# AtlasAnalyticsLab/AtlasPatch

Measured on AMD Instinct MI355X. Metric: patches/sec embedded (256x256, ViT-B/16), higher is better.
Workload: dtype f16

## Files before the change

atlaspatch_amd/csrc/ap_common.h:

```cpp
#pragma once
#include <hip/hip_runtime.h>
#include <cstdarg>
#include <cstdint>
#include <cstdio>
#include "../../include/atlaspatch_hip.h"

namespace ap {

void set_error(const char* fmt, ...);

#define AP_HIP_CHECK(expr)                                                              \
    do {                                                                                \
        hipError_t _e = (expr);                                                         \
        if (_e != hipSuccess) {                                                         \
            ap::set_error("%s failed: %s (%s:%d)", #expr, hipGetErrorString(_e),        \
                          __FILE__, __LINE__);                                          \
            return AP_ERR_HIP;                                                          \
        }                                                                               \
    } while (0)

#define AP_REQUIRE(cond, ...)                                                           \
    do {                                                                                \
        if (!(cond)) {                                                                  \
            ap::set_error(__VA_ARGS__);                                                 \
// ... 90 lines not shown
    int split;
    const float* resid; int ldr;
    int win_mode, win_ws, win_H, win_W, win_nwy, win_nwx;
    const float* zero_row;
};
void set_gemm_trace(long long* buf, int tiles_per_wg);

int launch_gemm(int dtype, int epilogue, const GemmArgs& a, hipStream_t stream);
int launch_gemm_impl(int dtype, int epilogue, const GemmArgs& a, int impl, int variant, hipStream_t stream);
bool gemm256_supports(int dtype, int epilogue, const GemmArgs& a);
int launch_gemm256(int dtype, int epilogue, const GemmArgs& a, int variant, hipStream_t stream);
int launch_gemm256_alt(int dtype, int epilogue, const GemmArgs& a, int variant, hipStream_t stream);

int launch_layernorm(int dtype, const float* x, long stride, int rows, int dim,
                     const float* gamma, const float* beta, float eps, void* out,
                     hipStream_t stream);
int launch_add_layernorm(int delta_dtype, int out_dtype, float* x, long stride, const void* delta,
                         long dstride, const float* ls, int rows, int dim, const float* gamma, const float* beta,
                         float eps, void* out, hipStream_t stream);
int launch_add2_layernorm(int delta_dtype, int out_dtype, float* x, long stride, const void* delta0, long dstride0,
                          const float* ls0, const void* delta1, long dstride1, const float* ls1, int store,
                          int rows, int dim, const float* gamma, const float* beta, float eps, void* out,
                          hipStream_t stream);
int launch_layernorm_f32out(const float* x, long stride, int rows, int dim, const float* gamma,
                            const float* beta, float eps, float* out, hipStream_t stream);
int launch_attention(int dtype, const void* qkv, void* out, int n, int tokens, int heads,
                     int head_dim, float scale, hipStream_t stream);
int launch_attention_flash(int dtype, const void* qkv, void* out, int n, int tokens, int heads, int head_dim, float scale,
                           hipStream_t stream);
int launch_attention_cls(int dtype, const void* q, const void* kv, int ld, int koff, int voff, void* out, int n,
                         int tokens, int heads, int head_dim, float scale, hipStream_t stream);
int launch_attn_pool(int dtype, const void* kv, const float* q, void* out, int n, int tokens, int heads,
                     hipStream_t stream);
int launch_stream_init(int dtype, const float* tok, int rows, int dim, float eps, void* x, float* rowstats,
                       hipStream_t stream);
int launch_rowstats_finalize(const float* partial, int rows, int groups, int dim, float eps, float* rowstats,
                             hipStream_t stream);
int launch_rowstats_finalize_cls(const float* partial, int rows, int groups, int dim, float eps, float* rowstats, int dtype,
                                 float* cls32, const float* branch, void* x, int n, int tokens, hipStream_t stream);
int launch_stream_to_f32(int dtype, const void* x, long stride, int rows, int dim, float* dst, hipStream_t stream);
int launch_rope(int dtype, void* qkv, int n, int tokens, int prefix, int heads, int head_dim, const float* cos, const float* sin,
                int which, hipStream_t stream);
int launch_cls_mean_pool(const float* y, int n, int tokens, int prefix, int dim, float* out, hipStream_t stream);
int launch_fold_ln(int dtype, const float* w32, int rows, int cols, int ld, const float* gamma, const float* beta,
                   const float* bias_in, void* wout, float* colsum, float* bias_out, hipStream_t stream, int swiglu_h = 0);
int launch_fold_ls(int dtype, const float* w32, int rows, int cols, int ld, const float* ls, const float* bias_in,
                   void* wout, float* bias_out, hipStream_t stream);
int launch_cls_stream(int dtype, const float* prefix, int prefix_rows, int img_rows, int n, int tokens, int dim, void* x, float* partial,
                      hipStream_t stream);
int launch_cls_init(float* tok, const float* prefix, int prefix_rows, int n, int tokens, int dim, hipStream_t stream);
int launch_cls_exact_update(int dtype, float* cls32, const float* branch, int n, int tokens, int dim, void* x, float* partial,
                            hipStream_t stream);
int launch_swiglu(int dtype, const void* x, int rows, int h, void* out, hipStream_t stream);
int launch_prefix_build(const float* cls, const float* reg, int reg_rows, const float* pos, int dim, float* prefix, hipStream_t stream);
int launch_convert(int dtype, const float* src, void* dst, size_t count, hipStream_t stream);
int launch_split_f16_weights(const float* src, void* dst, size_t count, hipStream_t stream);
int launch_chw_to_patchrows(int x_dtype, int dtype, const void* x, int n, int S, int ps, void* dst,
                            int ld, hipStream_t stream);

bool sattention_supports(int heads, int tq, int tk, int d, long ldq, long ldk, long ldv, long ldo);
int launch_sattention(const float* q, long ldq, const float* k, long ldk, const float* v, long ldv, int batch, int heads, int tq,
                      int tk, int d, float scale, float* out, long ldo, hipStream_t stream, bool exact);

int launch_conv2d_nhwc(int dtype, const void* x, int n, int h, int w, int cin, const void* weight, const float* bias, int cout,
                       int ksize, int stride, int pad, const void* resid, int relu, void* out, hipStream_t stream);
int launch_preproc_nhwc8(const uint8_t* src, int n, int h, int w, int top, int left, int S, const float mean[3],
// ... 27 lines not shown
```

atlaspatch_amd/csrc/vit.cpp:

```cpp
#include <cmath>
#include <cstdlib>
#include <cstring>
#include <map>
#include <string>
#include <vector>
#include "engine_host.h"

namespace ap {

struct Param {
    size_t count = 0;
    int rows = 0, cols = 0, ld = 0;
    bool matrix = false;
    void* dev = nullptr;
    float* dev32 = nullptr;
    void* split = nullptr;
    bool set = false;
};

struct BlockParams {
    const float *ln1_w, *ln1_b, *qkv_b, *proj_b, *ln2_w, *ln2_b, *fc1_b, *fc2_b, *ls1, *ls2;
    const Param *qkv, *proj, *fc1, *fc2;
};
struct FusedBlock {
    void *qkv_w = nullptr, *fc1_w = nullptr, *proj_w = nullptr, *fc2_w = nullptr;
    float *qkv_cs = nullptr, *qkv_b = nullptr, *fc1_cs = nullptr, *fc1_b = nullptr, *proj_b = nullptr, *fc2_b = nullptr;
};
struct PoolParams {
    const float *ln_k_w, *ln_k_b, *kv_b, *q, *out_b, *ln_out_w, *ln_out_b;
    const Param *kv, *out;
};
}

struct ap_vit {
    ap_vit_config cfg;
    int grid = 0, patches = 0, tokens = 0, kpe = 0;
    int prefix = 1;
    int pos_rows = 0, pos_row0 = 1;
    int hd = 64, dattn = 0;
    int fc1_rows = 0;
    float attn_scale = 0.125f;
    float* prefix_dev = nullptr;
    std::map<std::string, ap::Param> params;
    bool finalized = false;
    std::vector<ap::BlockParams> blocks;
    ap::PoolParams pool{};
    const ap::Param* pe_w = nullptr;
    const float *pe_b = nullptr, *cls = nullptr, *pos = nullptr, *norm_w = nullptr, *norm_b = nullptr;
    const float *pre_w = nullptr, *pre_b = nullptr;
    const float *rope_cos = nullptr, *rope_sin = nullptr;
    const ap::Param* head_proj = nullptr;
    float* zero_bias = nullptr;
    bool full_last_block = false, two_half_overlap = false, f32_stream = false;
    bool exact_cls = true;
    bool split_f16 = false;
    std::vector<ap::FusedBlock> fused;
    std::vector<void*> fused_allocs;
    void* pos16 = nullptr;
    bool fold_dirty = false;
    std::vector<float*> pending_free;
    int device = 0;
    ap::LaunchProfiler prof;
    hipStream_t side = nullptr;
    hipEvent_t ev_fork = nullptr, ev_join = nullptr;

    ~ap_vit() {
        for (auto& kv : params) {
            if (kv.second.dev) (void)hipFree(kv.second.dev);
            if (kv.second.dev32) (void)hipFree(kv.second.dev32);
            if (kv.second.split) (void)hipFree(kv.second.split);
        }
        for (void* p : fused_allocs) (void)hipFree(p);
        if (prefix_dev) (void)hipFree(prefix_dev);
        if (zero_bias) (void)hipFree(zero_bias);
        if (ev_fork) (void)hipEventDestroy(ev_fork);
        if (ev_join) (void)hipEventDestroy(ev_join);
        if (side) (void)hipStreamDestroy(side);
    }
};

namespace {

using ap::Param;
using ap::ScopedTimer;

int alloc_param(ap_vit* m, const std::string& name, int rows, int cols, bool matrix) {
    Param p;
// ... 88 lines not shown
      if ((rc = ap::launch_gemm(dt, ap::EPI_PATCH_EMBED, g, stream)) != AP_OK) return rc; }
    return ap::launch_cls_init(w.tok, m->prefix_dev, m->prefix, n, m->tokens, D, stream);
}

int patch_embed_stream(ap_vit* m, int n, const Workspace& w, hipStream_t stream) {
    const ap_vit_config& c = m->cfg;
    const int dt = c.compute_dtype, D = c.dim;
    int rc;
    ap::GemmArgs g{};
    g.A = w.hid; g.lda = m->kpe; set_weight(m, g, m->pe_w);
    g.M = n * m->patches; g.N = D; g.K = m->kpe;
    g.bias = m->pe_b; g.pos16 = m->pos16; g.P = m->patches; g.R = m->prefix; g.pos_row0 = m->pos_row0;
    g.out = w.x16; g.ldo = D; g.partial = w.partial;
    { ScopedTimer t(m->prof, AP_PROF_GEMM_PATCH_EMBED, stream);
      if ((rc = ap::launch_gemm(dt, ap::EPI_PATCH_STREAM, g, stream)) != AP_OK) return rc; }
    ScopedTimer t(m->prof, AP_PROF_LAYERNORM, stream);
    if ((rc = ap::launch_cls_stream(dt, m->prefix_dev, m->prefix, 0, n, m->tokens, D, w.x16, w.partial, stream)) != AP_OK) return rc;
    return ap::launch_rowstats_finalize(w.partial, n * m->tokens, D / 64, D, c.ln_eps, w.rowstats, stream);
}

int block_attention(ap_vit* m, int n, const Workspace& w, hipStream_t stream) {
    const ap_vit_config& c = m->cfg;
    const int DA = m->dattn;
    ScopedTimer t(m->prof, AP_PROF_ATTENTION, stream);
    if (use_split(m) && n <= 65535) {
        const float* qp = (const float*)w.qkv;
        return ap::launch_sattention(qp, 3 * DA, qp + DA, 3 * DA, qp + 2 * DA, 3 * DA, n, c.heads, m->tokens, m->tokens, m->hd,
                                     m->attn_scale, (float*)w.att, DA, stream, false);
    }
    return ap::launch_attention(c.compute_dtype, w.qkv, w.att, n, m->tokens, c.heads, m->hd, m->attn_scale, stream);
}

int cls_tail_rows(ap_vit* m, int n, const Workspace& w, const ap::BlockParams& bp, long xn_stride, long tok_stride,
                  const void* pending, const float* pending_ls, long pending_stride, hipStream_t stream) {
    const ap_vit_config& c = m->cfg;
    const int dt = c.compute_dtype, D = c.dim, DA = m->dattn, H = c.mlp_dim, F1 = m->fc1_rows;
    const bool swiglu = c.mlp_type == AP_MLP_SWIGLU;
    int rc;
    char* q_cls = (char*)w.att;
    char* a_cls = (char*)w.att + (size_t)n * DA * ap::dtype_size(dt);
    {
        ap::GemmArgs g{};
        g.A = w.xn; g.lda = (int)xn_stride; set_weight(m, g, bp.qkv);
        g.M = n; g.N = DA; g.K = D; g.bias = bp.qkv_b; g.out = q_cls; g.ldo = DA;
        if ((rc = ap::launch_gemm_impl(dt, ap::EPI_BIAS_STORE, g, 128, 0, stream)) != AP_OK) return rc;
    }
    if ((rc = ap::launch_attention_cls(dt, q_cls, w.qkv, 3 * DA, DA, 2 * DA, a_cls, n, m->tokens, c.heads,
                                       m->hd, m->attn_scale, stream)) != AP_OK) return rc;
    {
        ap::GemmArgs g{};
        g.A = a_cls; g.lda = DA; set_weight(m, g, bp.proj);
        g.M = n; g.N = D; g.K = DA; g.bias = bp.proj_b; g.out = w.delta2; g.ldo = D;
        if ((rc = ap::launch_gemm_impl(dt, ap::EPI_BIAS_STORE, g, 128, 0, stream)) != AP_OK) return rc;
    }
    if ((rc = ap::launch_add2_layernorm(dt, dt, w.tok, tok_stride, pending, pending_stride, pending_ls, w.delta2, D,
                                        bp.ls1, 1, n, D, bp.ln2_w, bp.ln2_b, c.ln_eps, w.xn, stream)) != AP_OK)
        return rc;
    {
        ap::GemmArgs g{};
        g.A = w.xn; g.lda = D; set_weight(m, g, bp.fc1);
        g.M = n; g.N = F1; g.K = D; g.bias = bp.fc1_b; g.out = w.hid; g.ldo = F1;
        if ((rc = ap::launch_gemm_impl(dt, fc1_epilogue(c, false), g, 128, 0, stream)) != AP_OK) return rc;
        if (swiglu && (rc = ap::launch_swiglu(dt, w.hid, n, H, w.hid2, stream)) != AP_OK) return rc;
    }
    ap::GemmArgs g{};
    g.A = w.hid2; g.lda = H; set_weight(m, g, bp.fc2);
    g.M = n; g.N = D; g.K = H; g.bias = bp.fc2_b; g.out = w.delta; g.ldo = D;
    return ap::launch_gemm_impl(dt, ap::EPI_BIAS_STORE, g, 128, 0, stream);
}

int blocks_f32_stream(ap_vit* m, int n, const Workspace& w, StreamTail& st, hipStream_t stream) {
    const ap_vit_config& c = m->cfg;
    const int dt = c.compute_dtype, D = c.dim, M = n * m->tokens;
    const int DA = m->dattn, H = c.mlp_dim, F1 = m->fc1_rows;
    const bool swiglu = c.mlp_type == AP_MLP_SWIGLU;
    int rc;
    const void* pending = nullptr;
    long pending_stride = D;
    const bool cls_tail = c.pool == AP_POOL_CLS && !m->full_last_block;
    const float* pending_ls = nullptr;
    for (int i = 0; i < c.depth; ++i) {
// ... 60 lines not shown
    st.pending_stride = cls_tail ? pending_stride : (long)m->tokens * D;
    return AP_OK;
}

int blocks_fused(ap_vit* m, int n, const Workspace& w, StreamTail& st, hipStream_t stream) {
    const ap_vit_config& c = m->cfg;
    const int dt = c.compute_dtype, D = c.dim, M = n * m->tokens, G = D / 64;
    const int DA = m->dattn, H = c.mlp_dim, F1 = m->fc1_rows;
    const bool swiglu = c.mlp_type == AP_MLP_SWIGLU;
    int rc;
    const bool cls_tail = c.pool == AP_POOL_CLS && !m->full_last_block;
    const bool exact_cls = m->exact_cls && (c.pool == AP_POOL_CLS || c.pool == AP_POOL_CLS_MEAN) && M < (1 << 24);
    const long cls_stride = (long)m->tokens;
    if (exact_cls) {
        ScopedTimer t(m->prof, AP_PROF_CLS_TAIL, stream);
        if (c.pre_norm) {
            AP_HIP_CHECK(hipMemcpy2DAsync(w.cls32, (size_t)D * 4, w.tok, (size_t)cls_stride * D * 4, (size_t)D * 4, n,
                                          hipMemcpyDeviceToDevice, stream));
        } else if ((rc = ap::launch_cls_init(w.cls32, m->prefix_dev, 1, n, 1, D, stream)) != AP_OK) return rc;
    }
    auto exact_cls_update = [&]() -> int {
        ScopedTimer t(m->prof, AP_PROF_LAYERNORM, stream);
        return ap::launch_cls_exact_update(dt, w.cls32, w.cls_branch, n, m->tokens, D, w.x16, w.partial, stream);
    };
    auto finalize_stats = [&]() -> int {
        ScopedTimer t(m->prof, AP_PROF_LAYERNORM, stream);
        return ap::launch_rowstats_finalize_cls(w.partial, M, G, D, c.ln_eps, w.rowstats, dt, exact_cls ? w.cls32 : nullptr,
                                                w.cls_branch, w.x16, n, m->tokens, stream);
    };
    for (int i = 0; i < c.depth; ++i) {
        const ap::BlockParams& bp = m->blocks[i];
        const ap::FusedBlock& fb = m->fused[i];
        const bool tail = i == c.depth - 1 && cls_tail;
        {
            const int col0 = tail ? DA : 0;
            ap::GemmArgs g{};
            g.A = w.x16; g.lda = D; set_weight(m, g, bp.qkv, col0, fb.qkv_w);
            g.M = M; g.N = 3 * DA - col0; g.K = D; g.bias = fb.qkv_b + col0; g.colsum = fb.qkv_cs + col0; g.rowstats = w.rowstats;
            g.out = (char*)w.qkv + (size_t)col0 * ap::dtype_size(dt); g.ldo = 3 * DA;
            ScopedTimer t(m->prof, AP_PROF_GEMM_QKV, stream);
            if ((rc = ap::launch_gemm(dt, ap::EPI_NORM_STORE, g, stream)) != AP_OK) return rc;
            if (c.rope && (rc = ap::launch_rope(dt, w.qkv, n, m->tokens, m->prefix, c.heads, m->hd, m->rope_cos, m->rope_sin,
                                                tail ? 2 : 3, stream)) != AP_OK) return rc;
        }
        if (tail) {
            ScopedTimer t(m->prof, AP_PROF_CLS_TAIL, stream);
            if (exact_cls) AP_HIP_CHECK(hipMemcpyAsync(w.tok, w.cls32, (size_t)n * D * 4, hipMemcpyDeviceToDevice, stream));
            else if ((rc = ap::launch_stream_to_f32(dt, w.x16, (long)m->tokens * D, n, D, w.tok, stream)) != AP_OK) return rc;
            if ((rc = ap::launch_add2_layernorm(dt, dt, w.tok, D, nullptr, 0, nullptr, nullptr, 0, nullptr, 0,
                                                n, D, bp.ln1_w, bp.ln1_b, c.ln_eps, w.xn, stream)) != AP_OK) return rc;
            if ((rc = cls_tail_rows(m, n, w, bp, D, D, nullptr, nullptr, 0, stream)) != AP_OK) return rc;
            st.pending = w.delta; st.pending_ls = bp.ls2; st.pending_stride = D; st.tok_stride = D;
            return AP_OK;
        }
        if ((rc = block_attention(m, n, w, stream)) != AP_OK) return rc;
        {
            ap::GemmArgs g{};
            g.A = w.att; g.lda = DA; set_weight(m, g, bp.proj, 0, fb.proj_w);
            g.M = M; g.N = D; g.K = DA; g.bias = fb.proj_b; g.out = w.x16; g.ldo = D; g.partial = w.partial;
            if (exact_cls) { g.cls_branch = w.cls_branch; g.cls_tokens = m->tokens; }
            ScopedTimer t(m->prof, AP_PROF_GEMM_PROJ, stream);
            if ((rc = ap::launch_gemm(dt, ap::EPI_RESID_STATS, g, stream)) != AP_OK) return rc;
        }
        if ((rc = finalize_stats()) != AP_OK) return rc;
        {
            ap::GemmArgs g{};
            g.A = w.x16; g.lda = D; set_weight(m, g, bp.fc1, 0, fb.fc1_w);
            g.M = M; g.N = F1; g.K = D; g.bias = fb.fc1_b; g.colsum = fb.fc1_cs; g.rowstats = w.rowstats;
            g.out = swiglu ? w.hid2 : w.hid; g.ldo = swiglu ? H : F1;
            ScopedTimer t(m->prof, AP_PROF_GEMM_FC1, stream);
            if ((rc = ap::launch_gemm(dt, fc1_epilogue(c, true), g, stream)) != AP_OK) return rc;
        }
        {
            ap::GemmArgs g{};
            g.A = w.hid2; g.lda = H; set_weight(m, g, bp.fc2, 0, fb.fc2_w);
            g.M = M; g.N = D; g.K = H; g.bias = fb.fc2_b; g.out = w.x16; g.ldo = D; g.partial = w.partial;
            if (exact_cls) { g.cls_branch = w.cls_branch; g.cls_tokens = m->tokens; }
            ScopedTimer t(m->prof, AP_PROF_GEMM_FC2, stream);
            if ((rc = ap::launch_gemm(dt, ap::EPI_RESID_STATS, g, stream)) != AP_OK) return rc;
        }
        if (i + 1 < c.depth) { if ((rc = finalize_stats()) != AP_OK) return rc; }
        else if (exact_cls && (rc = exact_cls_update()) != AP_OK) return rc;
    }
    if ((rc = ap::launch_stream_to_f32(dt, w.x16, D, M, D, w.tok, stream)) != AP_OK) return rc;
// ... 138 lines not shown
               "vit_create: compute dtype %d", c.compute_dtype);
    AP_REQUIRE(c.pool == AP_POOL_CLS || c.pool == AP_POOL_ATTN || c.pool == AP_POOL_CLS_MEAN, "vit_create: pool %d", c.pool);
    if (c.pool == AP_POOL_ATTN) {
        AP_REQUIRE(c.compute_dtype != AP_F32, "vit_create: the attentional pooler runs in float16 / bfloat16 only");
        AP_REQUIRE(c.pool_heads > 0 && c.pool_dim == c.pool_heads * 64 && c.pool_dim % 128 == 0 &&
                   2 * c.pool_dim <= c.mlp_dim && 2 * c.pool_dim <= 3 * c.dim,
                   "vit_create: pool_dim %d / pool_heads %d (heads of 64, multiple of 128)", c.pool_dim, c.pool_heads);
    }
    AP_REQUIRE(c.rope == 0 || (c.head_dim == 0 || c.head_dim * c.heads == c.dim), "vit_create: rope needs the true head width");
    AP_REQUIRE(c.act == AP_ACT_GELU || (c.act == AP_ACT_QUICK_GELU && c.mlp_type == AP_MLP_GELU), "vit_create: act %d", c.act);
    AP_REQUIRE(c.proj_dim == 0 || (c.pool == AP_POOL_CLS && c.proj_dim % 128 == 0 && c.proj_dim <= c.dim),
               "vit_create: proj_dim %d (class-token pooling, a multiple of 128, at most dim)", c.proj_dim);
    const int g = c.image_size / c.patch_size;
    const int prefix = 1 + c.reg_tokens;
    AP_REQUIRE(c.compute_dtype != AP_F32 || (prefix + g * g <= 288 && hd == 64),
               "vit_create: %d tokens / head width %d exceed the float32 attention kernel's limits (288 tokens, 64 wide); use "
               "float16 / bfloat16", prefix + g * g, hd);
    int device = 0;
    AP_HIP_CHECK(hipGetDevice(&device));
    ap_vit* m = new ap_vit();
    m->cfg = c;
    m->device = device;
    m->grid = g; m->patches = g * g; m->prefix = prefix; m->tokens = prefix + g * g;
    m->pos_rows = c.no_embed_class ? g * g : m->tokens;
    m->pos_row0 = c.no_embed_class ? 0 : prefix;
    m->hd = hd; m->dattn = c.heads * hd;
    m->attn_scale = c.attn_scale > 0.f ? c.attn_scale : 1.0f / sqrtf((float)hd);
    m->fc1_rows = c.mlp_type == AP_MLP_SWIGLU ? 2 * c.mlp_dim : c.mlp_dim;
    m->kpe = (int)ap::align_up(3 * c.patch_size * c.patch_size, 64);
    m->full_last_block = getenv("AP_VIT_FULL_LAST_BLOCK") != nullptr;
    m->two_half_overlap = getenv("AP_VIT_OVERLAP") != nullptr;
    m->f32_stream = getenv("AP_VIT_F32_STREAM") != nullptr;
    m->exact_cls = getenv("AP_VIT_NO_EXACT_CLS") == nullptr;
    m->split_f16 = c.compute_dtype == AP_F32 && getenv("AP_VIT_EXACT_F32") == nullptr;
    auto add = [&](const std::string& name, int rows, int cols, bool matrix) {
        if (rc == AP_OK) rc = alloc_param(m, name, rows, cols, matrix);
    };
    const int D = c.dim;
    add("patch_embed.weight", D, 3 * c.patch_size * c.patch_size, true);
    add("patch_embed.bias", 1, D, false);
    add("cls_token", 1, D, false);
    if (c.reg_tokens > 0) add("reg_tokens", c.reg_tokens, D, false);
    add("pos_embed", m->pos_rows, D, false);
    add("norm.weight", 1, D, false);
    add("norm.bias", 1, D, false);
    if (c.pre_norm) { add("pre_norm.weight", 1, D, false); add("pre_norm.bias", 1, D, false); }
    if (c.rope) { add("rope.cos", m->patches, hd, false); add("rope.sin", m->patches, hd, false); }
    if (c.proj_dim > 0) {
        add("head_proj.weight", c.proj_dim, D, true);
        if (rc == AP_OK && (hipMalloc((void**)&m->zero_bias, (size_t)c.proj_dim * sizeof(float)) != hipSuccess ||
                            hipMemset(m->zero_bias, 0, (size_t)c.proj_dim * sizeof(float)) != hipSuccess)) {
            ap::set_error("vit_create: hipMalloc of the projection's zero bias failed");
            rc = AP_ERR_HIP;
        }
    }
    for (int i = 0; i < c.depth; ++i) {
        const std::string b = "blocks." + std::to_string(i) + ".";
        add(b + "ln1.weight", 1, D, false); add(b + "ln1.bias", 1, D, false);
        add(b + "qkv.weight", 3 * m->dattn, D, true); add(b + "qkv.bias", 1, 3 * m->dattn, false);
        add(b + "proj.weight", D, m->dattn, true); add(b + "proj.bias", 1, D, false);
        add(b + "ln2.weight", 1, D, false); add(b + "ln2.bias", 1, D, false);
        add(b + "fc1.weight", m->fc1_rows, D, true); add(b + "fc1.bias", 1, m->fc1_rows, false);
        add(b + "fc2.weight", D, c.mlp_dim, true); add(b + "fc2.bias", 1, D, false);
        if (c.layer_scale) { add(b + "ls1", 1, D, false); add(b + "ls2", 1, D, false); }
    }
    if (c.pool == AP_POOL_ATTN) {
// ... 165 lines not shown
            for (const Param* p : {bp.qkv, bp.proj, bp.fc1, bp.fc2})
                if (!p->dev32) { ap::set_error("vit_finalize: block %d: a block parameter (or pos_embed) changed after a finalize -- the LayerNorm / LayerScale folding needs the float32 values of all four matrices of every block again: upload qkv / proj / fc1 / fc2 weights before finalizing", i); return AP_ERR_STATE; }
            fb.qkv_w = dalloc((size_t)3 * DA * bp.qkv->ld * es); fb.qkv_cs = (float*)dalloc(3 * DA * 4); fb.qkv_b = (float*)dalloc(3 * DA * 4);
            fb.fc1_w = dalloc((size_t)F1 * bp.fc1->ld * es); fb.fc1_cs = (float*)dalloc(F1 * 4); fb.fc1_b = (float*)dalloc(F1 * 4);
            fb.proj_w = dalloc((size_t)D * bp.proj->ld * es); fb.proj_b = (float*)dalloc(D * 4);
            fb.fc2_w = dalloc((size_t)D * bp.fc2->ld * es); fb.fc2_b = (float*)dalloc(D * 4);
            if (rc != AP_OK) break;
            if ((rc = ap::launch_fold_ln(dt, bp.qkv->dev32, 3 * DA, D, bp.qkv->ld, bp.ln1_w, bp.ln1_b, bp.qkv_b, fb.qkv_w, fb.qkv_cs, fb.qkv_b, nullptr)) != AP_OK) break;
            if ((rc = ap::launch_fold_ln(dt, bp.fc1->dev32, F1, D, bp.fc1->ld, bp.ln2_w, bp.ln2_b, bp.fc1_b, fb.fc1_w, fb.fc1_cs, fb.fc1_b, nullptr,
                                         m->cfg.mlp_type == AP_MLP_SWIGLU ? H : 0)) != AP_OK) break;
            if ((rc = ap::launch_fold_ls(dt, bp.proj->dev32, D, DA, bp.proj->ld, bp.ls1, bp.proj_b, fb.proj_w, fb.proj_b, nullptr)) != AP_OK) break;
            if ((rc = ap::launch_fold_ls(dt, bp.fc2->dev32, D, H, bp.fc2->ld, bp.ls2, bp.fc2_b, fb.fc2_w, fb.fc2_b, nullptr)) != AP_OK) break;
        }
        if (rc == AP_OK) {
            m->pos16 = dalloc((size_t)m->pos_rows * D * es);
            if (rc == AP_OK) rc = ap::launch_convert(dt, m->pos, m->pos16, (size_t)m->pos_rows * D, nullptr);
        }
        if (rc != AP_OK) return rc;
        AP_HIP_CHECK(hipDeviceSynchronize());
        for (auto& kv : m->params)
            if (kv.second.dev32) { (void)hipFree(kv.second.dev32); kv.second.dev32 = nullptr; }
    }
    m->fold_dirty = false;
    m->finalized = true;
    return AP_OK;
}

int ap_vit_set_option(ap_vit* m, int option, int value) {
    AP_REQUIRE(m, "vit_set_option: null handle");
    if (option == AP_VIT_OPT_FULL_LAST_BLOCK) m->full_last_block = value != 0;
    else if (option == AP_VIT_OPT_TWO_HALF_OVERLAP) m->two_half_overlap = value != 0;
    else if (option == AP_VIT_OPT_F32_STREAM) m->f32_stream = value != 0;
    else if (option == AP_VIT_OPT_EXACT_CLS) m->exact_cls = value != 0;
    else if (option == AP_VIT_OPT_SPLIT_F16) {
        AP_REQUIRE(value == 0 || m->cfg.compute_dtype == AP_F32, "vit_set_option: AP_VIT_OPT_SPLIT_F16 is a mode of the float32 compute type");
        if (value != 0) { const int rc = build_split(m); if (rc != AP_OK) return rc; }
        m->split_f16 = value != 0;
    }
    else { ap::set_error("vit_set_option: unknown option %d", option); return AP_ERR_INVALID; }
    return AP_OK;
}

size_t ap_vit_workspace_bytes(const ap_vit* m, int n) {
    if (!m || n <= 0) return 0;
    const size_t whole = carve(m, n, nullptr).total;
    const int na = (n + 1) / 2;
    const size_t halves = carve(m, na, nullptr).total + (n - na > 0 ? carve(m, n - na, nullptr).total : 0);
    return whole > halves ? whole : halves;
}

int ap_vit_embed_dim(const ap_vit* m) {
    if (!m) return 0;
    if (m->cfg.proj_dim > 0) return m->cfg.proj_dim;
    return m->cfg.pool == AP_POOL_ATTN ? m->cfg.pool_dim : (m->cfg.pool == AP_POOL_CLS_MEAN ? 2 * m->cfg.dim : m->cfg.dim);
}

int ap_vit_profile_enable(ap_vit* m, int on) { return ap::profile_enable(m ? &m->prof : nullptr, "vit", on); }

int ap_vit_profile_read(ap_vit* m, double* ms_by_kind, long long* launches_by_kind, int kinds) {
    return ap::profile_read(m ? &m->prof : nullptr, "vit", AP_PROF_KINDS, ms_by_kind, launches_by_kind, kinds);
}

int ap_vit_forward_u8(ap_vit* m, const uint8_t* patches, int n, int h, int w, const float mean[3],
                      const float stdv[3], float* out, void* workspace, size_t workspace_bytes,
                      ap_stream_t stream) {
    int rc = ap::check_forward_args("vit", m, n, patches && out, workspace, workspace_bytes, ap_vit_workspace_bytes);
// ... 54 lines not shown
```

atlaspatch_amd/encoders/vit.py:

```python
from __future__ import annotations

import ctypes as C
import re
import logging
import os
from pathlib import Path
from typing import Optional

import numpy as np
import torch

from .. import _lib
from .base import HipViTFeatureExtractor, NativeEncoder

logger = logging.getLogger("atlaspatch_amd.encoders.vit")

IMAGENET_MEAN = (0.485, 0.456, 0.406)
IMAGENET_STD = (0.229, 0.224, 0.225)
OPENAI_CLIP_MEAN = (0.48145466, 0.4578275, 0.40821073)
OPENAI_CLIP_STD = (0.26862954, 0.26130258, 0.27577711)

TRANSFORM_RESIZE = {
    "vit_b_16": (256, "bilinear"),
    "vit_b_32": (256, "bilinear"),
# ... 475 lines not shown
                             1 if attn_pool else (2 if cls_mean else 0), int(arch.get("pool_dim", 0)), int(arch.get("pool_heads", 0)),
                             float(arch.get("pool_ln_eps", 1e-5)),
                             int(arch.get("reg_tokens", 0)), 1 if arch.get("no_embed_class") else 0,
                             1 if arch.get("mlp") == "swiglu" else 0, hd_stored,
                             0.0 if hd_stored == hd_true else float(1.0 / np.sqrt(np.float32(hd_true))),
                             1 if arch.get("pre_norm") else 0, 1 if arch.get("act") == "quick_gelu" else 0,
                             int(arch.get("proj_dim", 0)), 1 if arch.get("rope") else 0)
        state = pad_heads(state, dim=arch["dim"], heads=arch["heads"], depth=arch["depth"])
        state = pad_mlp(state, mlp_dim=arch["mlp_dim"], depth=arch["depth"], swiglu=arch.get("mlp") == "swiglu")
        self._open(cfg, state)

    def _upload(self, arrs: dict) -> None:
        n = len(arrs)
        names = (C.c_char_p * n)(*[k.encode() for k in arrs])
        ptrs = (C.c_void_p * n)(*[a.ctypes.data for a in arrs.values()])
        counts = (C.c_size_t * n)(*[a.size for a in arrs.values()])
        _lib.check(self.lib.ap_vit_set_params(self._handle, names, ptrs, counts, n), "ap_vit_set_params")

    def forward_chw(self, x: torch.Tensor, out: Optional[torch.Tensor] = None) -> torch.Tensor:
        self._live()
        assert x.is_contiguous() and x.dim() == 4
        n = x.shape[0]
        if out is None:
            out = torch.empty((n, self.embed_dim), dtype=torch.float32, device=self.device)
        if n == 0:
            return out
        ws = self._ws(n)
        with torch.cuda.device(self.device):
            _lib.check(self.lib.ap_vit_forward_chw(self._handle, x.data_ptr(), _lib.torch_dtype_code(x.dtype), n,
                                                   out.data_ptr(), ws.data_ptr(), ws.numel(),
                                                   _lib.current_stream_ptr(self.device)), "ap_vit_forward_chw")
        return out

    OPTIONS = {"full_last_block": 0, "two_half_overlap": 1, "f32_stream": 2, "exact_cls": 3, "split_f16": 4}

    def set_option(self, name: str, on: bool) -> None:
        value = int(on) if not isinstance(on, bool) else (1 if on else 0)
        _lib.check(self.lib.ap_vit_set_option(self._handle, self.OPTIONS[name], value), "ap_vit_set_option")


def weights_path(name: str) -> Optional[Path]:
    root = os.environ.get("ATLASPATCH_WEIGHTS_DIR")
    if not root:
        return None
    for ext in (".safetensors", ".pt", ".pth"):
        candidate = Path(root) / f"{name}{ext}"
        if candidate.exists():
            return candidate
    return None


def load_checkpoint(path: Path) -> dict:
    if path.suffix == ".safetensors":
        from safetensors.torch import load_file
        return load_file(str(path))
    obj = torch.load(str(path), map_location="cpu", weights_only=True)
    for key in ("model", "state_dict"):
        if isinstance(obj, dict) and key in obj and isinstance(obj[key], dict):
            obj = obj[key]
    return obj


def resolve_weights(name: str, state_dict: Optional[dict], random_init_seed: Optional[int], random_init,
                    key_families: str) -> tuple[dict, bool]:
    if state_dict is not None:
        return state_dict, False
    path = weights_path(name)
# ... 124 lines not shown
```

include/atlaspatch_hip.h:

```cpp
#ifndef ATLASPATCH_HIP_H
#define ATLASPATCH_HIP_H

#include <stddef.h>
#include <stdint.h>

#ifdef __cplusplus
extern "C" {
#endif

#define AP_OK 0
#define AP_ERR_INVALID (-1)
#define AP_ERR_HIP (-2)
#define AP_ERR_WORKSPACE (-3)
#define AP_ERR_UNSUPPORTED (-4)
#define AP_ERR_STATE (-5)
#define AP_ERR_CAPACITY (-6)

#define AP_F32 0
#define AP_F16 1
#define AP_BF16 2

typedef void* ap_stream_t;

#define AP_ABI_VERSION 20
// ... 66 lines not shown
    int reg_tokens;
    int no_embed_class;
    int mlp_type;
    int head_dim;
    float attn_scale;
    int pre_norm;
    int act;
    int proj_dim;
    int rope;
} ap_vit_config;
#define AP_VIT_CONFIG_SIZE_V20 92u
size_t ap_sizeof_vit_config(void);
int ap_vit_config_init(ap_vit_config* cfg, size_t sizeof_caller);
#define AP_ACT_GELU 0
#define AP_ACT_QUICK_GELU 1
#define AP_MLP_GELU 0
#define AP_MLP_SWIGLU 1
#define AP_POOL_CLS 0
#define AP_POOL_ATTN 1
#define AP_POOL_CLS_MEAN 2

int ap_vit_create(const ap_vit_config* cfg, ap_vit** out);
void ap_vit_destroy(ap_vit* m);

int ap_vit_set_param(ap_vit* m, const char* name, const float* host, size_t count);
int ap_vit_set_params(ap_vit* m, const char* const* names, const float* const* host, const size_t* counts, int n);
int ap_vit_finalize(ap_vit* m);

#define AP_VIT_OPT_FULL_LAST_BLOCK 0
#define AP_VIT_OPT_TWO_HALF_OVERLAP 1
#define AP_VIT_OPT_F32_STREAM 2
#define AP_VIT_OPT_EXACT_CLS 3
#define AP_VIT_OPT_SPLIT_F16 4
int ap_vit_set_option(ap_vit* m, int option, int value);

size_t ap_vit_workspace_bytes(const ap_vit* m, int n);
int ap_vit_embed_dim(const ap_vit* m);

#define AP_PROF_PREPROC 0
#define AP_PROF_GEMM_PATCH_EMBED 1
#define AP_PROF_GEMM_QKV 2
#define AP_PROF_GEMM_PROJ 3
#define AP_PROF_GEMM_FC1 4
#define AP_PROF_GEMM_FC2 5
#define AP_PROF_ATTENTION 6
#define AP_PROF_LAYERNORM 7
#define AP_PROF_CLS_TAIL 8
#define AP_PROF_KINDS 9
int ap_vit_profile_enable(ap_vit* m, int on);
int ap_vit_profile_read(ap_vit* m, double* ms_by_kind, long long* launches_by_kind, int kinds);

int ap_vit_forward_u8(ap_vit* m, const uint8_t* patches, int n, int h, int w,
                      const float mean[3], const float stdv[3],
                      float* out, void* workspace, size_t workspace_bytes, ap_stream_t stream);

int ap_vit_forward_chw(ap_vit* m, const void* x, int x_dtype, int n,
                       float* out, void* workspace, size_t workspace_bytes, ap_stream_t stream);

#define AP_EPI_BIAS 0
#define AP_EPI_BIAS_GELU 1
#define AP_EPI_BIAS_RESID 2
#define AP_EPI_BIAS_QUICK_GELU 10
int ap_gemm(int dtype, int epilogue, const void* A, int lda, const void* W, int ldw,
            int M, int N, int K, const float* bias, const float* gamma, void* out, int ldo,
            int impl, int variant, ap_stream_t stream);
int ap_split_f16_weights(const float* w32, void* out, size_t count, ap_stream_t stream);
// ... 221 lines not shown
```

Measured before the change: 30540.

## Compute last-block CLS attention directly from LN-folded stream, skipping K/V GEMM

For the final block, when only the CLS token's output is needed, the change skips the full K/V projection GEMM over all tokens. Instead it folds the query into the key weights (u = q·Wk), scores tokens directly against the normalized residual stream using row stats, and forms a softmax-weighted sum of the stream. That sum is then projected through Wv. This replaces an O(tokens·D·2DA) GEMM with per-image reductions, at the cost of new custom kernels and a fp32 workspace that reuses the hid and qkv buffers.

```diff
diff --git a/atlaspatch_amd/csrc/ap_common.h b/atlaspatch_amd/csrc/ap_common.h
--- a/atlaspatch_amd/csrc/ap_common.h
+++ b/atlaspatch_amd/csrc/ap_common.h
@@ -146,6 +146,20 @@
                          int tokens, int heads, int head_dim, float scale, hipStream_t stream);
 int launch_attn_pool(int dtype, const void* kv, const float* q, void* out, int n, int tokens, int heads,
                      hipStream_t stream);
+struct ClsReadoutArgs {
+    const void* q;
+    const void* x;
+    const float* rowstats;
+    const void* wkv; int ldw;
+    const float *cs_kv, *b_kv;
+    float *u, *z;
+    float *qcs, *c;
+    void* out;
+    int n, tokens, heads, head_dim, dim;
+    float scale;
+};
+bool cls_readout_supports(int dtype, int tokens, int heads, int head_dim, int dim);
+int launch_cls_readout(int dtype, const ClsReadoutArgs& a, hipStream_t stream);
 int launch_stream_init(int dtype, const float* tok, int rows, int dim, float eps, void* x, float* rowstats,
                        hipStream_t stream);
 int launch_rowstats_finalize(const float* partial, int rows, int groups, int dim, float eps, float* rowstats,
diff --git a/atlaspatch_amd/csrc/cls_readout.hip b/atlaspatch_amd/csrc/cls_readout.hip
--- /dev/null
+++ b/atlaspatch_amd/csrc/cls_readout.hip
@@ -0,0 +1,289 @@
+#include "ap_common.h"
+
+namespace ap {
+namespace {
+
+template <typename T> struct Vec;
+template <> struct Vec<f16> { using v8 = f16x8; using v4 = f16x4; };
+template <> struct Vec<bf16> { using v8 = bf16x8; using v4 = bf16x4; };
+
+constexpr int kImg = 8;
+constexpr int kHC = 12;
+constexpr int kTileRows = 64, kTileCols = 128;
+constexpr int kTileLd = kTileCols + 8;
+
+template <typename T>
+__global__ __launch_bounds__(128) void cls_u_kernel(const T* __restrict__ q, const T* __restrict__ wk, int ldw,
+                                                    const float* __restrict__ csk, float* __restrict__ u,
+                                                    float* __restrict__ qcs, int n, int heads, int hd, int D) {
+    using V8 = typename Vec<T>::v8;
+    __shared__ float qs[kImg][128];
+    const int img0 = blockIdx.x * kImg, h = blockIdx.y, DA = heads * hd;
+    for (int idx = threadIdx.x; idx < kImg * hd; idx += 128) {
+        const int i = idx / hd, j = idx - i * hd;
+        qs[i][j] = img0 + i < n ? (float)q[(size_t)(img0 + i) * DA + h * hd + j] : 0.f;
+    }
+    __syncthreads();
+    const int d = (blockIdx.z * 128 + threadIdx.x) * 8;
+    if (d < D) {
+        float acc[kImg][8];
+#pragma unroll
+        for (int i = 0; i < kImg; ++i)
+#pragma unroll
+            for (int e = 0; e < 8; ++e) acc[i][e] = 0.f;
+        const T* wp = wk + (size_t)h * hd * ldw + d;
+        for (int j = 0; j < hd; ++j) {
+            const V8 w8 = *(const V8*)(wp + (size_t)j * ldw);
+            float wf[8];
+#pragma unroll
+            for (int e = 0; e < 8; ++e) wf[e] = (float)w8[e];
+#pragma unroll
+            for (int i = 0; i < kImg; ++i) {
+                const float qv = qs[i][j];
+#pragma unroll
+                for (int e = 0; e < 8; ++e) acc[i][e] = __builtin_fmaf(qv, wf[e], acc[i][e]);
+            }
+        }
+#pragma unroll
+        for (int i = 0; i < kImg; ++i)
+            if (img0 + i < n) {
+                float* up = u + ((size_t)(img0 + i) * heads + h) * D + d;
+                *(f32x4*)up = f32x4{acc[i][0], acc[i][1], acc[i][2], acc[i][3]};
+                *(f32x4*)(up + 4) = f32x4{acc[i][4], acc[i][5], acc[i][6], acc[i][7]};
+            }
+    }
+    if (blockIdx.z == 0 && threadIdx.x < kImg && img0 + threadIdx.x < n) {
+        float s = 0.f;
+        for (int j = 0; j < hd; ++j) s = __builtin_fmaf(qs[threadIdx.x][j], csk[h * hd + j], s);
+        qcs[(size_t)(img0 + threadIdx.x) * heads + h] = s;
+    }
+}
+
+__device__ __forceinline__ float wave_sum(float v) {
+#pragma unroll
+    for (int off = 32; off > 0; off >>= 1) v += __shfl_xor(v, off, 64);
+    return v;
+}
+__device__ __forceinline__ float wave_max(float v) {
+#pragma unroll
+    for (int off = 32; off > 0; off >>= 1) v = fmaxf(v, __shfl_xor(v, off, 64));
+    return v;
+}
+
+template <typename T>
+__global__ __launch_bounds__(256) void cls_readout_kernel(const T* __restrict__ x, const float* __restrict__ rowstats,
+                                                          const float* __restrict__ u, const float* __restrict__ qcs,
+                                                          float* __restrict__ z, float* __restrict__ c, int tokens, int heads,
+                                                          int HP, int D, float scale) {
+    using V8 = typename Vec<T>::v8;
+    using V4 = typename Vec<T>::v4;
+    extern __shared__ __attribute__((aligned(16))) float sm[];
+    float* wgt = sm;
+    float* stats = sm + (size_t)tokens * HP + kHC;
+    T* tile = (T*)(stats + 2 * ((tokens + 1) & ~1));
+    float* red = (float*)tile;
+    const int img = blockIdx.x;
+    const T* xb = x + (size_t)img * tokens * D;
+    const int lane = threadIdx.x & 63;
+    const int wave = __builtin_amdgcn_readfirstlane(threadIdx.x >> 6);
+    for (int i = threadIdx.x; i < 2 * tokens; i += 256) stats[i] = rowstats[(size_t)img * tokens * 2 + i];
+
+    for (int h0 = 0; h0 < heads; h0 += kHC) {
+        const int nh = heads - h0 < kHC ? heads - h0 : kHC;
+        for (int t0 = 0; t0 < tokens; t0 += kTileRows) {
+            float part[kHC];
+#pragma unroll
+            for (int hh = 0; hh < kHC; ++hh) part[hh] = 0.f;
+            for (int c0 = 0; c0 < D; c0 += kTileCols) {
+                __syncthreads();
+#pragma unroll
+                for (int k = 0; k < 4; ++k) {
+                    const int o = threadIdx.x + k * 256, row = o >> 4, oc = o & 15, t = t0 + row;
+                    V8 v;
+#pragma unroll
+                    for (int e = 0; e < 8; ++e) v[e] = (T)0.f;
+                    if (t < tokens) v = *(const V8*)(xb + (size_t)t * D + c0 + oc * 8);
+                    *(V8*)(tile + row * kTileLd + oc * 8) = v;
+                }
+                __syncthreads();
+                const float* up = u + ((size_t)img * heads + h0) * D + c0 + wave * 32;
+#pragma unroll
+                for (int o = 0; o < 4; ++o) {
+                    const V8 v = *(const V8*)(tile + lane * kTileLd + wave * 32 + o * 8);
+                    float xf[8];
+#pragma unroll
+                    for (int e = 0; e < 8; ++e) xf[e] = (float)v[e];
+#pragma unroll
+                    for (int hh = 0; hh < kHC; ++hh)
+                        if (hh < nh) {
+                            const float* uh = up + (size_t)hh * D + o * 8;
+#pragma unroll
+                            for (int e = 0; e < 8; ++e) part[hh] = __builtin_fmaf(xf[e], uh[e], part[hh]);
+                        }
+                }
+            }
+            __syncthreads();
+#pragma unroll
+            for (int hh = 0; hh < kHC; ++hh) red[(wave * kHC + hh) * 64 + lane] = part[hh];
+            __syncthreads();
+            for (int idx = threadIdx.x; idx < 64 * nh; idx += 256) {
+                const int hh = idx >> 6, r = idx & 63, t = t0 + r;
+                if (t < tokens) {
+                    const float dot = (red[hh * 64 + r] + red[(kHC + hh) * 64 + r]) +
+                                      (red[(2 * kHC + hh) * 64 + r] + red[(3 * kHC + hh) * 64 + r]);
+                    const float s = __builtin_fmaf(stats[2 * t], dot, stats[2 * t + 1] * qcs[(size_t)img * heads + h0 + hh]);
+                    wgt[t * HP + h0 + hh] = s * scale;
+                }
+            }
+        }
+    }
+    __syncthreads();
+
+    for (int h = wave; h < heads; h += 4) {
+        float mx = -INFINITY;
+        for (int t = lane; t < tokens; t += 64) mx = fmaxf(mx, wgt[t * HP + h]);
+        mx = wave_max(mx);
+        float sum = 0.f;
+        for (int t = lane; t < tokens; t += 64) {
+            const float p = __expf(wgt[t * HP + h] - mx);
+            wgt[t * HP + h] = p;
+            sum += p;
+        }
+        sum = wave_sum(sum);
+        float cs = 0.f;
+        for (int t = lane; t < tokens; t += 64) {
+            const float p = wgt[t * HP + h] / sum;
+            cs = __builtin_fmaf(p, stats[2 * t + 1], cs);
+            wgt[t * HP + h] = p * stats[2 * t];
+        }
+        cs = wave_sum(cs);
+        if (lane == 0) c[(size_t)img * heads + h] = cs;
+    }
+    __syncthreads();
+
+    for (int h0 = 0; h0 < heads; h0 += kHC) {
+        const int nh = heads - h0 < kHC ? heads - h0 : kHC;
+        for (int q4 = threadIdx.x; q4 < D / 4; q4 += 256) {
+            float acc[kHC][4];
+#pragma unroll
+            for (int hh = 0; hh < kHC; ++hh)
+#pragma unroll
+                for (int e = 0; e < 4; ++e) acc[hh][e] = 0.f;
+            const T* xp = xb + q4 * 4;
+#pragma unroll 4
+            for (int t = 0; t < tokens; ++t) {
+                const V4 v = *(const V4*)(xp + (size_t)t * D);
+                const float* wt = wgt + t * HP + h0;
+#pragma unroll
+                for (int g = 0; g < kHC / 4; ++g) {
+                    const f32x4 p4 = *(const f32x4*)(wt + 4 * g);
+#pragma unroll
+                    for (int k = 0; k < 4; ++k)
+#pragma unroll
+                        for (int e = 0; e < 4; ++e) acc[4 * g + k][e] = __builtin_fmaf(p4[k], (float)v[e], acc[4 * g + k][e]);
+                }
+            }
+#pragma unroll
+            for (int hh = 0; hh < kHC; ++hh)
+                if (hh < nh)
+                    *(f32x4*)(z + ((size_t)img * heads + h0 + hh) * D + q4 * 4) = f32x4{acc[hh][0], acc[hh][1], acc[hh][2], acc[hh][3]};
+        }
+    }
+}
+
+template <typename T>
+__global__ __launch_bounds__(256) void cls_av_kernel(const float* __restrict__ z, const float* __restrict__ c,
+                                                     const T* __restrict__ wv, int ldw, const float* __restrict__ csv,
+                                                     const float* __restrict__ bv, T* __restrict__ out, int n, int heads, int hd,
+                                                     int D) {
+    using V8 = typename Vec<T>::v8;
+    __shared__ __attribute__((aligned(16))) float zs[kImg][128];
+    __shared__ float red[4][kImg][128];
+    const int img0 = blockIdx.x * kImg, h = blockIdx.y, DA = heads * hd;
+    const int parts = 256 / hd;
+    const int cp = 128 / parts;
+    const int part = threadIdx.x / hd, j = threadIdx.x - part * hd;
+    const bool active = part < parts;
+    float acc[kImg];
+#pragma unroll
+    for (int i = 0; i < kImg; ++i) acc[i] = 0.f;
+    for (int d0 = 0; d0 < D; d0 += 128) {
+        __syncthreads();
+        for (int idx = threadIdx.x; idx < kImg * 128; idx += 256) {
+            const int i = idx >> 7, d = idx & 127;
+            zs[i][d] = img0 + i < n ? z[((size_t)(img0 + i) * heads + h) * D + d0 + d] : 0.f;
+        }
+        __syncthreads();
+        if (active) {
+            const T* wr = wv + (size_t)(h * hd + j) * ldw + d0 + part * cp;
+            for (int o = 0; o < cp; o += 8) {
+                const V8 w8 = *(const V8*)(wr + o);
+                float wf[8];
+#pragma unroll
+                for (int e = 0; e < 8; ++e) wf[e] = (float)w8[e];
+#pragma unroll
+                for (int i = 0; i < kImg; ++i) {
+                    const f32x4 a = *(const f32x4*)&zs[i][part * cp + o], b = *(const f32x4*)&zs[i][part * cp + o + 4];
+#pragma unroll
+                    for (int e = 0; e < 4; ++e) acc[i] = __builtin_fmaf(a[e], wf[e], acc[i]);
+#pragma unroll
+                    for (int e = 0; e < 4; ++e) acc[i] = __builtin_fmaf(b[e], wf[4 + e], acc[i]);
+                }
+            }
+        }
+    }
+    if (active) {
+#pragma unroll
+        for (int i = 0; i < kImg; ++i) red[part][i][j] = acc[i];
+    }
+    __syncthreads();
+    for (int idx = threadIdx.x; idx < kImg * hd; idx += 256) {
+        const int i = idx / hd, jj = idx - i * hd;
+        if (img0 + i >= n) continue;
+        float dot = red[0][i][jj] + red[1][i][jj];
+        if (parts == 4) dot += red[2][i][jj] + red[3][i][jj];
+        const int col = h * hd + jj;
+        const float a = __builtin_fmaf(c[(size_t)(img0 + i) * heads + h], csv[col], dot) + bv[col];
+        out[(size_t)(img0 + i) * DA + col] = from_f32<T>(a);
+    }
+}
+
+size_t readout_lds_bytes(int tokens, int heads) {
+    const int HP = (heads + 3) & ~3;
+    return ((size_t)tokens * HP + kHC + 2 * (size_t)((tokens + 1) & ~1)) * sizeof(float) + (size_t)kTileRows * kTileLd * 2;
+}
+
+template <typename T>
+int launch_typed(const ClsReadoutArgs& a, hipStream_t stream) {
+    const int DA = a.heads * a.head_dim, HP = (a.heads + 3) & ~3;
+    const T* wk = (const T*)a.wkv;
+    const T* wv = wk + (size_t)DA * a.ldw;
+    cls_u_kernel<T><<<dim3((a.n + kImg - 1) / kImg, a.heads, (a.dim + 1023) / 1024), 128, 0, stream>>>(
+        (const T*)a.q, wk, a.ldw, a.cs_kv, a.u, a.qcs, a.n, a.heads, a.head_dim, a.dim);
+    AP_HIP_CHECK(hipGetLastError());
+    cls_readout_kernel<T><<<a.n, 256, readout_lds_bytes(a.tokens, a.heads), stream>>>(
+        (const T*)a.x, a.rowstats, a.u, a.qcs, a.z, a.c, a.tokens, a.heads, HP, a.dim, a.scale);
+    AP_HIP_CHECK(hipGetLastError());
+    cls_av_kernel<T><<<dim3((a.n + kImg - 1) / kImg, a.heads), 256, 0, stream>>>(
+        a.z, a.c, wv, a.ldw, a.cs_kv + DA, a.b_kv + DA, (T*)a.out, a.n, a.heads, a.head_dim, a.dim);
+    AP_HIP_CHECK(hipGetLastError());
+    return AP_OK;
+}
+
+}
+
+bool cls_readout_supports(int dtype, int tokens, int heads, int head_dim, int dim) {
+    return (dtype == AP_F16 || dtype == AP_BF16) && (head_dim == 64 || head_dim == 96 || head_dim == 128) && heads > 0 &&
+           heads <= 65535 && tokens > 0 && dim > 0 && dim % 128 == 0 && readout_lds_bytes(tokens, heads) <= 64 * 1024;
+}
+
+int launch_cls_readout(int dtype, const ClsReadoutArgs& a, hipStream_t stream) {
+    AP_REQUIRE(cls_readout_supports(dtype, a.tokens, a.heads, a.head_dim, a.dim),
+               "cls_readout: unsupported problem (dtype %d, %d tokens, %d heads of %d, dim %d)", dtype, a.tokens, a.heads, a.head_dim, a.dim);
+    AP_REQUIRE(a.q && a.x && a.rowstats && a.wkv && a.cs_kv && a.b_kv && a.u && a.qcs && a.z && a.c && a.out, "cls_readout: null pointer");
+    AP_REQUIRE(a.ldw >= a.dim && a.ldw % 8 == 0, "cls_readout: weight row stride %d", a.ldw);
+    if (a.n <= 0) return AP_OK;
+    return dtype == AP_F16 ? launch_typed<f16>(a, stream) : launch_typed<bf16>(a, stream);
+}
+
+}
diff --git a/atlaspatch_amd/csrc/vit.cpp b/atlaspatch_amd/csrc/vit.cpp
--- a/atlaspatch_amd/csrc/vit.cpp
+++ b/atlaspatch_amd/csrc/vit.cpp
@@ -53,6 +53,7 @@
     float* zero_bias = nullptr;
     bool full_last_block = false, two_half_overlap = false, f32_stream = false;
     bool exact_cls = true;
+    bool cls_readout = true;
     bool split_f16 = false;
     std::vector<ap::FusedBlock> fused;
     std::vector<void*> fused_allocs;
@@ -207,7 +208,8 @@
 }
 
 int cls_tail_rows(ap_vit* m, int n, const Workspace& w, const ap::BlockParams& bp, long xn_stride, long tok_stride,
-                  const void* pending, const float* pending_ls, long pending_stride, hipStream_t stream) {
+                  const void* pending, const float* pending_ls, long pending_stride, hipStream_t stream,
+                  const ap::FusedBlock* readout = nullptr) {
     const ap_vit_config& c = m->cfg;
     const int dt = c.compute_dtype, D = c.dim, DA = m->dattn, H = c.mlp_dim, F1 = m->fc1_rows;
     const bool swiglu = c.mlp_type == AP_MLP_SWIGLU;
@@ -220,8 +222,17 @@
         g.M = n; g.N = DA; g.K = D; g.bias = bp.qkv_b; g.out = q_cls; g.ldo = DA;
         if ((rc = ap::launch_gemm_impl(dt, ap::EPI_BIAS_STORE, g, 128, 0, stream)) != AP_OK) return rc;
     }
-    if ((rc = ap::launch_attention_cls(dt, q_cls, w.qkv, 3 * DA, DA, 2 * DA, a_cls, n, m->tokens, c.heads,
-                                       m->hd, m->attn_scale, stream)) != AP_OK) return rc;
+    if (readout) {
+        const size_t nhd = (size_t)n * c.heads * D;
+        ap::ClsReadoutArgs r{};
+        r.q = q_cls; r.x = w.x16; r.rowstats = w.rowstats;
+        r.wkv = (const char*)readout->qkv_w + (size_t)DA * bp.qkv->ld * ap::dtype_size(dt); r.ldw = bp.qkv->ld;
+        r.cs_kv = readout->qkv_cs + DA; r.b_kv = readout->qkv_b + DA;
+        r.u = (float*)w.hid; r.qcs = r.u + nhd; r.z = (float*)w.qkv; r.c = r.z + nhd;
+        r.out = a_cls; r.n = n; r.tokens = m->tokens; r.heads = c.heads; r.head_dim = m->hd; r.dim = D; r.scale = m->attn_scale;
+        if ((rc = ap::launch_cls_readout(dt, r, stream)) != AP_OK) return rc;
+    } else if ((rc = ap::launch_attention_cls(dt, q_cls, w.qkv, 3 * DA, DA, 2 * DA, a_cls, n, m->tokens, c.heads,
+                                              m->hd, m->attn_scale, stream)) != AP_OK) return rc;
     {
         ap::GemmArgs g{};
         g.A = a_cls; g.lda = DA; set_weight(m, g, bp.proj);
@@ -348,7 +359,11 @@
         const ap::BlockParams& bp = m->blocks[i];
         const ap::FusedBlock& fb = m->fused[i];
         const bool tail = i == c.depth - 1 && cls_tail;
-        {
+        const size_t readout_bytes = ((size_t)n * c.heads * D + (size_t)n * c.heads) * sizeof(float);
+        const bool readout = tail && m->cls_readout && !c.rope && ap::cls_readout_supports(dt, m->tokens, c.heads, m->hd, D) &&
+                             readout_bytes <= (size_t)M * H * ap::dtype_size(dt) &&
+                             readout_bytes <= (size_t)M * 3 * DA * ap::dtype_size(dt);
+        if (!readout) {
             const int col0 = tail ? DA : 0;
             ap::GemmArgs g{};
             g.A = w.x16; g.lda = D; set_weight(m, g, bp.qkv, col0, fb.qkv_w);
@@ -365,7 +380,7 @@
             else if ((rc = ap::launch_stream_to_f32(dt, w.x16, (long)m->tokens * D, n, D, w.tok, stream)) != AP_OK) return rc;
             if ((rc = ap::launch_add2_layernorm(dt, dt, w.tok, D, nullptr, 0, nullptr, nullptr, 0, nullptr, 0,
                                                 n, D, bp.ln1_w, bp.ln1_b, c.ln_eps, w.xn, stream)) != AP_OK) return rc;
-            if ((rc = cls_tail_rows(m, n, w, bp, D, D, nullptr, nullptr, 0, stream)) != AP_OK) return rc;
+            if ((rc = cls_tail_rows(m, n, w, bp, D, D, nullptr, nullptr, 0, stream, readout ? &fb : nullptr)) != AP_OK) return rc;
             st.pending = w.delta; st.pending_ls = bp.ls2; st.pending_stride = D; st.tok_stride = D;
             return AP_OK;
         }
@@ -570,6 +585,7 @@
     m->two_half_overlap = getenv("AP_VIT_OVERLAP") != nullptr;
     m->f32_stream = getenv("AP_VIT_F32_STREAM") != nullptr;
     m->exact_cls = getenv("AP_VIT_NO_EXACT_CLS") == nullptr;
+    m->cls_readout = getenv("AP_VIT_NO_CLS_READOUT") == nullptr;
     m->split_f16 = c.compute_dtype == AP_F32 && getenv("AP_VIT_EXACT_F32") == nullptr;
     auto add = [&](const std::string& name, int rows, int cols, bool matrix) {
         if (rc == AP_OK) rc = alloc_param(m, name, rows, cols, matrix);
@@ -801,6 +817,7 @@
     else if (option == AP_VIT_OPT_TWO_HALF_OVERLAP) m->two_half_overlap = value != 0;
     else if (option == AP_VIT_OPT_F32_STREAM) m->f32_stream = value != 0;
     else if (option == AP_VIT_OPT_EXACT_CLS) m->exact_cls = value != 0;
+    else if (option == AP_VIT_OPT_CLS_READOUT) m->cls_readout = value != 0;
     else if (option == AP_VIT_OPT_SPLIT_F16) {
         AP_REQUIRE(value == 0 || m->cfg.compute_dtype == AP_F32, "vit_set_option: AP_VIT_OPT_SPLIT_F16 is a mode of the float32 compute type");
         if (value != 0) { const int rc = build_split(m); if (rc != AP_OK) return rc; }
diff --git a/atlaspatch_amd/encoders/vit.py b/atlaspatch_amd/encoders/vit.py
--- a/atlaspatch_amd/encoders/vit.py
+++ b/atlaspatch_amd/encoders/vit.py
@@ -531,7 +531,8 @@
                                                    _lib.current_stream_ptr(self.device)), "ap_vit_forward_chw")
         return out
 
-    OPTIONS = {"full_last_block": 0, "two_half_overlap": 1, "f32_stream": 2, "exact_cls": 3, "split_f16": 4}
+    OPTIONS = {"full_last_block": 0, "two_half_overlap": 1, "f32_stream": 2, "exact_cls": 3, "split_f16": 4,
+               "cls_readout": 5}
 
     def set_option(self, name: str, on: bool) -> None:
         value = int(on) if not isinstance(on, bool) else (1 if on else 0)
diff --git a/include/atlaspatch_hip.h b/include/atlaspatch_hip.h
--- a/include/atlaspatch_hip.h
+++ b/include/atlaspatch_hip.h
@@ -122,6 +122,7 @@
 #define AP_VIT_OPT_F32_STREAM 2
 #define AP_VIT_OPT_EXACT_CLS 3
 #define AP_VIT_OPT_SPLIT_F16 4
+#define AP_VIT_OPT_CLS_READOUT 5
 int ap_vit_set_option(ap_vit* m, int option, int value);
 
 size_t ap_vit_workspace_bytes(const ap_vit* m, int n);
```

Result: no change. 30690 (median of 5 runs) (+0.5%).
